# maciejkula/sbr-rs

Hardware: AMD Instinct MI355X
Metric: train interactions/sec (higher is better)
Workload: dtype f32

## Files before the change

sbr_rs_amd/csrc/sbr_device.h:

```cpp
#ifndef SBR_DEVICE_H
#define SBR_DEVICE_H

#include <hip/hip_runtime.h>

#include "../../include/sbr_hip.h"
#include "sbr_kernels.h"
#include "sbr_numerics.h"

namespace sbr {

typedef float f32x16 __attribute__((ext_vector_type(16)));

__device__ __forceinline__ float4 ld4(const float* p) { return *reinterpret_cast<const float4*>(p); }
__device__ __forceinline__ void st4(float* p, float4 v) { *reinterpret_cast<float4*>(p) = v; }
typedef float v4f_nt __attribute__((ext_vector_type(4)));
__device__ __forceinline__ float4 ld4s(const float* p) {
    const v4f_nt v = __builtin_nontemporal_load(reinterpret_cast<const v4f_nt*>(p));
    return make_float4(v.x, v.y, v.z, v.w);
}
__device__ __forceinline__ void st4s(float* p, float4 v) {
    v4f_nt t; t.x = v.x; t.y = v.y; t.z = v.z; t.w = v.w;
    __builtin_nontemporal_store(t, reinterpret_cast<v4f_nt*>(p));
}

typedef unsigned v2u __attribute__((ext_vector_type(2)));
template <int CTRL>
__device__ __forceinline__ float dpp_read(float p) {
    return __uint_as_float(__builtin_amdgcn_update_dpp(0u, __float_as_uint(p), CTRL, 0xF, 0xF, true));
}
template <int L>
__device__ __forceinline__ float group_allreduce(float p) {
    if constexpr (L >= 64) {
        const v2u r = __builtin_amdgcn_permlane32_swap(__float_as_uint(p), __float_as_uint(p), false, false);
        p = __uint_as_float(r.x) + __uint_as_float(r.y);
    }
    if constexpr (L >= 32) {
        const v2u r = __builtin_amdgcn_permlane16_swap(__float_as_uint(p), __float_as_uint(p), false, false);
        p = __uint_as_float(r.x) + __uint_as_float(r.y);
    }
    if constexpr (L >= 16) p = p + dpp_read<0x128>(p);
    if constexpr (L >= 8) {
        unsigned t = __builtin_amdgcn_update_dpp(0u, __float_as_uint(p), 0x104, 0xF, 0x5, false);
        t = __builtin_amdgcn_update_dpp(t, __float_as_uint(p), 0x114, 0xF, 0xA, false);
        p = p + __uint_as_float(t);
    }
    if constexpr (L >= 4) p = p + dpp_read<0x4E>(p);
    if constexpr (L >= 2) p = p + dpp_read<0xB1>(p);
    return p;
}
__device__ __forceinline__ void opt_update(const ModelView& m, float* w, float* acc, float* mom, float g) {
    if (m.optimizer == SBR_OPT_ADAM) sbr_adam(w, mom, acc, g, m.lr, m.l2, m.c1, m.c2);
    else sbr_adagrad(w, acc, g, m.lr, m.l2);
}


template <int D>
struct LaneGroup {
    static constexpr int L = D / 4, GPW = 64 / L;
    int lg, grp;
    uint64_t wave_first, stride;
    __device__ __forceinline__ LaneGroup(uint64_t wave = (blockIdx.x * (uint64_t)blockDim.x + threadIdx.x) >> 6,
                                         uint64_t nwaves = ((uint64_t)gridDim.x * blockDim.x) >> 6)
        : lg((int)(threadIdx.x & 63) % L), grp((int)(threadIdx.x & 63) / L), wave_first(wave * GPW), stride(nwaves * GPW) {}
    __device__ __forceinline__ uint64_t first() const { return wave_first + grp; }
};

struct EntrySource {
    uint32_t r, kind;
    __device__ __forceinline__ const float* rows(const float* dX, const float* H) const { return kind == 0 ? dX : H; }
    __device__ __forceinline__ float scale(float c) const { return kind == 0 ? 1.0f : (kind == 1 ? -c : c); }
    __device__ __forceinline__ float scale_at(const float* coef) const { return kind == 0 ? 1.0f : scale(coef[r]); }
    __device__ __forceinline__ bool carries_bias() const { return kind != 0; }
};
__device__ __forceinline__ EntrySource entry_source(uint32_t key_lo) { return EntrySource{key_lo / 3, key_lo % 3}; }

struct SeenBools {
    bool empty, hb;
    __device__ __forceinline__ SeenBools(bool any_, bool has_b_) : empty(!any_), hb(has_b_) {}
    __device__ __forceinline__ bool any() const { return !empty; }
    __device__ __forceinline__ bool has_b() const { return hb; }
};
struct SeenWord {
    uint32_t w;
    __device__ __forceinline__ SeenWord(bool any_, bool has_b_) : w((any_ ? 1u : 0u) | (has_b_ ? 2u : 0u)) {}
    __device__ __forceinline__ bool any() const { return (w & 1u) != 0; }
    __device__ __forceinline__ bool has_b() const { return (w & 2u) != 0; }
};
template <class Seen>
struct RowSumT {
    float4 g;
    float gb;
    Seen seen;
    __device__ __forceinline__ RowSumT() : g(make_float4(0.f, 0.f, 0.f, 0.f)), gb(0.0f), seen(false, false) {}
    __device__ __forceinline__ RowSumT(float4 g_, float gb_, bool any_, bool has_b_) : g(g_), gb(gb_), seen(any_, has_b_) {}
    __device__ __forceinline__ RowSumT(float4 g_, float gb_, uint32_t fl) : RowSumT(g_, gb_, (fl & 1u) != 0, (fl & 2u) != 0) {}
    __device__ __forceinline__ bool any() const { return seen.any(); }
    __device__ __forceinline__ bool has_b() const { return seen.has_b(); }
    __device__ __forceinline__ uint32_t flags() const { return (any() ? 1u : 0u) | (has_b() ? 2u : 0u); }
    __device__ __forceinline__ void add_entry(float4 v, float scale, bool carries_bias) { *this = with_entry(*this, v, scale, carries_bias); }
    template <class S2>
    __device__ __forceinline__ void add_partial(const RowSumT<S2>& o) { *this = with_partial(*this, o.g, o.gb, o.any(), o.has_b()); }

private:
    static __device__ __forceinline__ RowSumT with_entry(const RowSumT& s, float4 v, float scale, bool carries_bias) {
        float4 g = s.g;
        float gb = s.gb;
        bool empty = !s.any(), has_b = s.has_b();
        if (empty) {
            g = make_float4(scale * v.x, scale * v.y, scale * v.z, scale * v.w);
            empty = false;
        } else {
            g.x = g.x + scale * v.x; g.y = g.y + scale * v.y;
            g.z = g.z + scale * v.z; g.w = g.w + scale * v.w;
        }
        if (carries_bias) {
            gb = has_b ? gb + scale : scale;
            has_b = true;
        }
        return RowSumT(g, gb, !empty, has_b);
    }
    static __device__ __forceinline__ RowSumT with_partial(const RowSumT& s, float4 v, float vb, bool o_any, bool o_has_b) {
        float4 g = s.g;
        float gb = s.gb;
        bool empty = !s.any(), has_b = s.has_b();
        if (o_any) {
            if (empty) g = v;
            else { g.x = g.x + v.x; g.y = g.y + v.y; g.z = g.z + v.z; g.w = g.w + v.w; }
            empty = false;
        }
        if (o_has_b) {
            gb = has_b ? gb + vb : vb;
            has_b = true;
        }
        return RowSumT(g, gb, !empty, has_b);
    }
};
typedef RowSumT<SeenBools> RowSum;
typedef RowSumT<SeenWord> RowSumW;

struct PlainAccess {
    static __device__ __forceinline__ float4 ld(const float* p) { return ld4(p); }
    static __device__ __forceinline__ void st(float* p, float4 v) { st4(p, v); }
};

template <int D, bool ADAGRAD_ONLY = false>
struct RowUpdate {
    float4 w, a, mo;
    float bv, ba, bmo;
    __device__ __forceinline__ RowUpdate() : w(make_float4(0.f, 0.f, 0.f, 0.f)), a(w), mo(w), bv(0.0f), ba(0.0f), bmo(0.0f) {}
    static __device__ __forceinline__ bool adam(const ModelView& m) { return !ADAGRAD_ONLY && m.optimizer == SBR_OPT_ADAM; }
    static __device__ __forceinline__ void element(const ModelView& m, float* wv, float* acc, float* mom, float g) {
        if constexpr (ADAGRAD_ONLY) sbr_adagrad(wv, acc, g, m.lr, m.l2);
        else opt_update(m, wv, acc, mom, g);
    }
    template <class Access = PlainAccess>
    __device__ __forceinline__ void load(const ModelView& m, uint64_t row, int lg) {
        w = Access::ld(m.E + row * D + 4 * lg);
        a = Access::ld(m.Eacc + row * D + 4 * lg);
        if (adam(m)) mo = ld4(m.Em + row * D + 4 * lg);
    }
    __device__ __forceinline__ void load_bias(const ModelView& m, uint64_t row) {
        bv = m.b[row]; ba = m.bacc[row];
        if (adam(m)) bmo = m.bm[row];
    }
    template <class Sum>
    __device__ __forceinline__ void apply(const ModelView& m, const Sum& s) {
        element(m, &w.x, &a.x, &mo.x, s.g.x);
        element(m, &w.y, &a.y, &mo.y, s.g.y);
        element(m, &w.z, &a.z, &mo.z, s.g.z);
        element(m, &w.w, &a.w, &mo.w, s.g.w);
    }
    template <class Sum>
    __device__ __forceinline__ void apply_bias(const ModelView& m, const Sum& s) { element(m, &bv, &ba, &bmo, s.gb); }
    template <class Access = PlainAccess>
    __device__ __forceinline__ void store(const ModelView& m, uint64_t row, int lg) const {
        Access::st(m.E + row * D + 4 * lg, w);
        Access::st(m.Eacc + row * D + 4 * lg, a);
        if (adam(m)) st4(m.Em + row * D + 4 * lg, mo);
    }
    __device__ __forceinline__ void store_bias(const ModelView& m, uint64_t row) const {
        m.b[row] = bv;
        m.bacc[row] = ba;
        if (adam(m)) m.bm[row] = bmo;
    }
    template <class Sum>
    __device__ __forceinline__ void update_bias(const ModelView& m, uint64_t row, int lg, const Sum& s) {
        if (lg != 0 || !s.has_b()) return;
        load_bias(m, row);
        apply_bias(m, s);
        store_bias(m, row);
    }
};

template <class T>
__device__ __forceinline__ T* launder(T* p) {
    typedef T __attribute__((address_space(1))) * global_ptr;
    global_ptr g = (global_ptr)p;
    asm volatile("" : "+s"(g));
    return (T*)g;
}

__device__ __forceinline__ float dot4(float4 x, float4 y) {
    float p = x.x * y.x;
    p = sbr_fma(x.y, y.y, p);
    p = sbr_fma(x.z, y.z, p);
    p = sbr_fma(x.w, y.w, p);
    return p;
}

typedef float v2f __attribute__((ext_vector_type(2)));
__device__ __forceinline__ v2f pk_fma(v2f a, v2f b, v2f c) { return __builtin_elementwise_fma(a, b, c); }
__device__ __forceinline__ v2f pk_splat(float x) { return (v2f){x, x}; }
__device__ __forceinline__ void tanh_pq_x2(v2f x, v2f* p, v2f* q) {
    const float cx = __builtin_amdgcn_fmed3f(x.x, -SBR_TANH_CLAMP, SBR_TANH_CLAMP), cy = __builtin_amdgcn_fmed3f(x.y, -SBR_TANH_CLAMP, SBR_TANH_CLAMP);
    x.x = x.x != x.x ? x.x : cx;
    x.y = x.y != x.y ? x.y : cy;
    const v2f x2 = x * x;
    v2f n = pk_splat(-2.76076847742355e-16f);
    n = pk_fma(n, x2, pk_splat(2.00018790482477e-13f));
    n = pk_fma(n, x2, pk_splat(-8.60467152213735e-11f));
    n = pk_fma(n, x2, pk_splat(5.12229709037114e-08f));
    n = pk_fma(n, x2, pk_splat(1.48572235717979e-05f));
    n = pk_fma(n, x2, pk_splat(6.37261928875436e-04f));
    n = pk_fma(n, x2, pk_splat(4.89352455891786e-03f));
    *p = n * x;
    v2f dq = pk_splat(1.19825839466702e-06f);
    dq = pk_fma(dq, x2, pk_splat(1.18534705686654e-04f));
    dq = pk_fma(dq, x2, pk_splat(2.26843463243900e-03f));
    dq = pk_fma(dq, x2, pk_splat(4.89352518554385e-03f));
    *q = dq;
}

__device__ __forceinline__ void phase_sync() {
    __builtin_amdgcn_fence(__ATOMIC_RELEASE, "workgroup");
    __syncthreads();
    __builtin_amdgcn_fence(__ATOMIC_ACQUIRE, "workgroup");
}

template <int NT>
__device__ __forceinline__ void small_tail(const MbView& mb, const BlockView& blk, const WorkView& w, const SmallTail& t, double lsum,
                                           unsigned int tsum) {
    constexpr int NMAX = 3 * SBR_SMALL_TAIL_MAX_ROWS, NW = NT / 64;
    __shared__ uint64_t ka[NMAX], kb[NMAX];
    __shared__ uint32_t s_cnt[NW];
    const int tid = threadIdx.x, lane = tid & 63, wave = tid >> 6;
    const int R = mb.R;
    const uint32_t n = 3u * (uint32_t)R;
    __builtin_amdgcn_fence(__ATOMIC_RELEASE, "agent");
    __syncthreads();
    __builtin_amdgcn_fence(__ATOMIC_ACQUIRE, "agent");
    if (wave == 0) {
        const int ns = mb.steps[0];
        const float x = t.lag_state[1 + 2 * (ns - 1)];
        float sum = 0.0f;
        for (int base = 0; base < ns; base += 64) {
            const int tt = base + lane;
            const float v = tt < ns ? w.loss[mb.off[tt]] : 0.0f;
            const int cnt = ns - base < 64 ? ns - base : 64;
            float mine = 0.0f;
            for (int l = 0; l < cnt; ++l) {
                sum = sum + __uint_as_float(__builtin_amdgcn_readlane(__float_as_uint(v), l));
                mine = lane == l ? sum : mine;
            }
            if (tt < ns) t.lag_state[1 + 2 * tt] = mine;
        }
        if (lane == 0) {
            t.header[0] = (uint32_t)R;
            t.header[1] = tsum;
            t.header[2] = t.header[3] = 0;
            *reinterpret_cast<double*>(t.header + 4) = lsum;
            *reinterpret_cast<unsigned long long*>(t.header + 6) = (unsigned long long)R;
            if (t.loss_acc) {
                t.loss_acc[0] += lsum;
                t.loss_acc[1] += lsum;
                t.ex_acc[0] += (unsigned long long)R;
                t.ex_acc[1] += tsum;
                t.ex_acc[2] += (unsigned long long)R;
            }
            t.lag_state[0] = t.lag_state[0] + x;
        }
    }
    for (uint32_t e = tid; e < n; e += NT) {
        const uint32_t r = e / 3u, kind = e - 3u * r;
        const uint32_t* a = kind == 0 ? blk.in_idx : (kind == 1 ? blk.out_idx : blk.neg);
        ka[e] = ((uint64_t)a[r] << 32) | e;
    }
    __syncthreads();
    for (uint32_t e = tid; e < n; e += NT) {
        const uint64_t k = ka[e];
        uint32_t rank = 0;
        for (uint32_t j = 0; j < n; ++j) rank += ka[j] < k ? 1u : 0u;
        kb[rank] = k;
    }
    __syncthreads();
    const uint64_t lt = (1ull << lane) - 1ull;
    uint32_t base_heads = 0;
    for (uint32_t p0 = 0; p0 < n; p0 += NT) {
        const uint32_t p = p0 + tid;
        const bool valid = p < n;
        const bool head = valid && (p == 0 || (uint32_t)(kb[p] >> 32) != (uint32_t)(kb[p - 1] >> 32));
        if (valid) t.keys_sorted[p] = kb[p];
        const uint64_t mm = __ballot(head);
        if (lane == 0) s_cnt[wave] = (uint32_t)__popcll(mm);
        __syncthreads();
        uint32_t off = base_heads, total = 0;
#pragma unroll
        for (int w2 = 0; w2 < NW; ++w2) {
            if (w2 < wave) off += s_cnt[w2];
            total += s_cnt[w2];
        }
        if (head) t.head_pos[off + (uint32_t)__popcll(mm & lt)] = p;
        base_heads += total;
        __syncthreads();
    }
    if (tid == 0) {
        *t.nheads = base_heads;
        t.head_pos[base_heads] = n;
    }
}

}

#define DISPATCH_D(d, ...)                                         \
    switch (d) {                                                   \
        case 16: { constexpr int DD = 16; __VA_ARGS__; } break;    \
        case 32: { constexpr int DD = 32; __VA_ARGS__; } break;    \
        case 64: { constexpr int DD = 64; __VA_ARGS__; } break;    \
        case 128: { constexpr int DD = 128; __VA_ARGS__; } break;  \
        case 256: { constexpr int DD = 256; __VA_ARGS__; } break;  \
        default: break;                                            \
    }
#define DISPATCH_NQ(ndev, ...)                                           \
    do {                                                                 \
        if ((ndev) <= 4) { constexpr int NQ = 4; __VA_ARGS__; }          \
        else if ((ndev) <= 8) { constexpr int NQ = 8; __VA_ARGS__; }     \
        else { constexpr int NQ = 16; __VA_ARGS__; }                     \
    } while (0)
#endif
```

sbr_rs_amd/csrc/sbr_kernels.hip:

```cpp

#include "sbr_kernels.h"

#include <atomic>
#include <cstdlib>
#include <cstring>

#include "../../include/sbr_hip.h"
#include "sbr_device.h"
#include "sbr_numerics.h"

namespace sbr {

typedef float f32x4 __attribute__((ext_vector_type(4)));
typedef unsigned v4u32 __attribute__((ext_vector_type(4)));

#define EWMA_CHUNK_SEQS 256
#ifndef SBR_FWD_RT
#define SBR_FWD_RT 4
#endif
#ifndef SBR_FWD_WPE
#define SBR_FWD_WPE 3
#endif
#define SBR_MAX_T 1024
#ifndef SBR_FWD_RT4_MIN_TILES
// ... 1748 lines not shown
    const int nslabs = (nr + SLAB - 1) / SLAB;
    float bias_acc = 0.0f;
    const bool do_bias = tk == 0 && tid < 128;
    fetch(0);
    for (int slab = 0; slab < nslabs; ++slab) {
#pragma unroll
        for (int i = 0; i < NI; ++i) {
            st4(&Xs[(srow + 8 * i) * 128 + c4], xr[i]);
            st4(&Zs[(srow + 8 * i) * 128 + c4], zr[i]);
        }
        __syncthreads();
        fetch(slab + 1 < nslabs ? slab + 1 : slab);
        const float* xa = &Xs[hh * 128 + wk * 64 + l31];
        const float* zb = &Zs[hh * 128 + wj * 64 + l31];
        float a0 = xa[0], a1 = xa[32], b0 = zb[0], b1 = zb[32];
#pragma unroll
        for (int s = 0; s < SLAB / 2; ++s) {
            const int sn = s + 1 < SLAB / 2 ? s + 1 : s;
            const float na0 = xa[sn * 256], na1 = xa[sn * 256 + 32];
            const float nb0 = zb[sn * 256], nb1 = zb[sn * 256 + 32];
            acc[0][0] = __builtin_amdgcn_mfma_f32_32x32x2f32(a0, b0, acc[0][0], 0, 0, 0);
            acc[0][1] = __builtin_amdgcn_mfma_f32_32x32x2f32(a0, b1, acc[0][1], 0, 0, 0);
            acc[1][0] = __builtin_amdgcn_mfma_f32_32x32x2f32(a1, b0, acc[1][0], 0, 0, 0);
            acc[1][1] = __builtin_amdgcn_mfma_f32_32x32x2f32(a1, b1, acc[1][1], 0, 0, 0);
            a0 = na0; a1 = na1; b0 = nb0; b1 = nb1;
        }
        if (do_bias) {
            const int rows_here = nr - slab * SLAB < SLAB ? nr - slab * SLAB : SLAB;
            for (int r = 0; r < rows_here; ++r) bias_acc = bias_acc + Zs[r * 128 + tid];
        }
        __syncthreads();
    }
    if (do_bias) w.partials[((size_t)c * (K2 + 1) + K2) * NGD + tj * 128 + tid] = bias_acc;
    float* part = w.partials + (size_t)c * (K2 + 1) * NGD;
#pragma unroll
    for (int a = 0; a < 2; ++a)
#pragma unroll
        for (int b = 0; b < 2; ++b) {
            const int j = tj * 128 + wj * 64 + b * 32 + l31;
#pragma unroll
            for (int q = 0; q < 16; ++q) {
                const int k = tk * 128 + wk * 64 + a * 32 + (q & 3) + 8 * (q >> 2) + 4 * hh;
                part[(size_t)k * NGD + j] = acc[a][b][q];
            }
        }
}

__global__ void dense_reduce_local_kernel(const float* partials, int nchunks, size_t n, float* dense) {
    const size_t i = (size_t)blockIdx.x * blockDim.x + threadIdx.x;
    if (i >= n) return;
    float acc = partials[i];
    int c = 1;
    for (; c + 8 <= nchunks; c += 8) {
        float v[8];
#pragma unroll
        for (int j = 0; j < 8; ++j) v[j] = partials[(size_t)(c + j) * n + i];
#pragma unroll
        for (int j = 0; j < 8; ++j) acc = acc + v[j];
    }
    for (; c < nchunks; ++c) acc = acc + partials[(size_t)c * n + i];
    dense[i] = acc;
}

__device__ __forceinline__ size_t wp_index(int k, int jcol, int D, int NG) {
    const int K2 = 2 * D;
    const int g = jcol / D, u = jcol % D;
    const int ut = u >> 4, j16 = u & 15;
    const int S = k >> 4, sub = (k & 15) >> 2, kq = k & 3;
    const int lane = kq * 16 + j16;
    return ((((size_t)(ut * NG + g) * (K2 / 16) + S) * 64 + lane) * 4 + sub);
}
__device__ __forceinline__ size_t wtp_index(int k, int jcol, int D, int NG) {
    const int NGD = NG * D;
    const int ct = k >> 4, c16 = k & 15;
    const int S = jcol >> 4, sub = (jcol & 15) >> 2, kq = jcol & 3;
    const int lane = kq * 16 + c16;
    return ((((size_t)ct * (NGD / 16) + S) * 64 + lane) * 4 + sub);
}

__device__ __forceinline__ void dense_apply_element(const ModelView& m, size_t i, float g);
__global__ void dense_apply_kernel(ModelView m, const uint8_t* all_blocks, uint64_t block_bytes, uint64_t dense_off,
                                   int ndev, size_t n, const float* partials, int nchunks, float* dense_out) {
    const size_t i = (size_t)blockIdx.x * blockDim.x + threadIdx.x;
    if (i >= n) return;
    float g;
    if (partials) {
        g = partials[i];
        int c = 1;
        for (; c + 8 <= nchunks; c += 8) {
            float v[8];
#pragma unroll
            for (int j = 0; j < 8; ++j) v[j] = partials[(size_t)(c + j) * n + i];
#pragma unroll
            for (int j = 0; j < 8; ++j) g = g + v[j];
        }
        for (; c < nchunks; ++c) g = g + partials[(size_t)c * n + i];
        dense_out[i] = g;
    } else {
        g = reinterpret_cast<const float*>(all_blocks + dense_off)[i];
        for (int q = 1; q < ndev; ++q) g = g + reinterpret_cast<const float*>(all_blocks + (size_t)q * block_bytes + dense_off)[i];
    }
    dense_apply_element(m, i, g);
}
__device__ __forceinline__ void dense_apply_element(const ModelView& m, size_t i, float g) {
    if (m.ng) {
        const int NGD = m.ng * m.d;
        const size_t nw = (size_t)2 * m.d * NGD;
        if (i < nw) {
            const bool adam = m.optimizer == SBR_OPT_ADAM;
            float wv = m.W[i], G = m.Wacc[i], M = adam ? m.Wm[i] : 0.0f;
            opt_update(m, &wv, &G, &M, g);
            m.W[i] = wv;
            m.Wacc[i] = G;
            if (adam) m.Wm[i] = M;
            const int k = (int)(i / NGD), jcol = (int)(i % NGD);
            m.Wp[wp_index(k, jcol, m.d, m.ng)] = wv;
            m.WTp[wtp_index(k, jcol, m.d, m.ng)] = wv;
        } else {
            const size_t j = i - nw;
            const bool adam = m.optimizer == SBR_OPT_ADAM;
            float wv = m.bW[j], G = m.bWacc[j], M = adam ? m.bWm[j] : 0.0f;
            opt_update(m, &wv, &G, &M, g);
            m.bW[j] = wv;
            m.bWacc[j] = G;
            if (adam) m.bWm[j] = M;
        }
    } else {
        const bool adam = m.optimizer == SBR_OPT_ADAM;
        float wv = m.alpha[i], G = m.alpha_acc[i], M = adam ? m.alpha_m[i] : 0.0f;
        opt_update(m, &wv, &G, &M, g);
        m.alpha[i] = wv;
        m.alpha_acc[i] = G;
        if (adam) m.alpha_m[i] = M;
    }
}

__global__ void repack_lstm_kernel(ModelView m) {
    const int NGD = m.ng * m.d;
    const size_t nw = (size_t)2 * m.d * NGD;
    const size_t i = (size_t)blockIdx.x * blockDim.x + threadIdx.x;
    if (i >= nw) return;
    const int k = (int)(i / NGD), jcol = (int)(i % NGD);
    const float wv = m.W[i];
    m.Wp[wp_index(k, jcol, m.d, m.ng)] = wv;
    m.WTp[wtp_index(k, jcol, m.d, m.ng)] = wv;
}


struct UpdAccess {
    static __device__ __forceinline__ float4 ld(const float* p) { return ld4_upd(p); }
    static __device__ __forceinline__ void st(float* p, float4 v) { st4_upd(p, v); }
};
struct NoPrefetch {};
struct EmitApply {
    ModelView m;
    template <int D>
    __device__ __forceinline__ RowUpdate<D> pre(uint32_t r, int lg) const {
        RowUpdate<D> q;
        q.template load<UpdAccess>(m, r, lg);
        return q;
    }
    template <int D>
    __device__ __forceinline__ void row(uint32_t r, uint64_t, int lg, const RowSum& s, RowUpdate<D> q) const {
        q.apply(m, s);
        q.template store<UpdAccess>(m, r, lg);
        q.update_bias(m, r, lg, s);
    }
};
struct EmitChunk {
    void* send;
    uint64_t S;
    template <int D>
    __device__ __forceinline__ NoPrefetch pre(uint32_t, int) const { return NoPrefetch{}; }
    template <int D>
    __device__ __forceinline__ void row(uint32_t r, uint64_t, int lg, const RowSum& s, NoPrefetch) const {
        const uint32_t S32 = (uint32_t)S, owner = r / S32;
        float* c = reinterpret_cast<float*>(send) + (uint64_t)owner * S * ((uint64_t)D + 2);
        const uint64_t lr = r - owner * S32;
        st4(c + lr * D + 4 * lg, s.g);
        if (lg == 0) {
            if (s.has_b()) c[S * D + lr] = s.gb;
            reinterpret_cast<uint32_t*>(c + S * D + S)[lr] = 1u | (s.has_b() ? 2u : 0u);
        }
    }
};
struct EmitList {
    float* G;
    float* gbl;
    uint32_t* fl;
    template <int D>
    __device__ __forceinline__ NoPrefetch pre(uint32_t, int) const { return NoPrefetch{}; }
    template <int D>
    __device__ __forceinline__ void row(uint32_t, uint64_t p, int lg, const RowSum& s, NoPrefetch) const {
        st4(G + p * D + 4 * lg, s.g);
        if (lg == 0) {
            gbl[p] = s.gb;
            fl[p] = 1u | (s.has_b() ? 2u : 0u);
        }
    }
};

template <int D>
__device__ __forceinline__ RowSum seg_accumulate(const BlockView& blk, const uint64_t* keys, uint64_t begin, uint64_t end, int lg) {
    RowSum s;
    for (uint64_t e = begin; e < end; e += 4) {
        float4 v[4];
        float sc[4];
        bool bias[4];
#pragma unroll
        for (int i = 0; i < 4; ++i) {
            v[i] = make_float4(0.f, 0.f, 0.f, 0.f);
            sc[i] = 0.0f;
            bias[i] = false;
            if (e + i < end) {
                const EntrySource src = entry_source((uint32_t)keys[e + i]);
                v[i] = ld4(src.rows(blk.dX, blk.H) + (size_t)src.r * D + 4 * lg);
                sc[i] = src.scale_at(blk.coef);
                bias[i] = src.carries_bias();
            }
        }
#pragma unroll
        for (int i = 0; i < 4; ++i)
            if (e + i < end) s.add_entry(v[i], sc[i], bias[i]);
    }
    return s;
}

template <int D, int NB>
__device__ __forceinline__ RowSum seg_accumulate_long(const BlockView& blk, const uint64_t* keys, uint64_t begin, uint64_t end, int lg) {
    RowSum s;
    const uint32_t* klo = reinterpret_cast<const uint32_t*>(keys);
    uint32_t src_n[NB];
#pragma unroll
    for (int i = 0; i < NB; ++i) src_n[i] = begin + i < end ? klo[2 * (begin + i)] : 0u;
#pragma unroll 1
    for (uint64_t e = begin; e < end; e += NB) {
        float4 v[NB];
        float sc[NB];
        EntrySource src[NB];
#pragma unroll
        for (int i = 0; i < NB; ++i) {
            src[i] = entry_source(src_n[i]);
            v[i] = make_float4(0.f, 0.f, 0.f, 0.f);
            sc[i] = 0.0f;
            if (e + i < end) {
                v[i] = ld4(src[i].rows(blk.dX, blk.H) + (size_t)src[i].r * D + 4 * lg);
                sc[i] = blk.coef[src[i].r];
            }
        }
#pragma unroll
        for (int i = 0; i < NB; ++i) src_n[i] = e + NB + i < end ? klo[2 * (e + NB + i)] : 0u;
#pragma unroll
        for (int i = 0; i < NB; ++i)
            if (e + i < end) s.add_entry(v[i], src[i].scale(sc[i]), src[i].carries_bias());
    }
    return s;
}

__device__ __forceinline__ uint64_t seg_end(const uint64_t* keys, uint64_t lo, uint64_t hi, uint32_t row) {
    while (lo < hi) {
        const uint64_t mid = lo + (hi - lo) / 2;
        if ((uint32_t)(keys[mid] >> 32) == row) lo = mid + 1; else hi = mid;
    }
    return lo;
}

template <int D, class Emit, bool INLINE_LONG>
__device__ __forceinline__ void seg_short_rows(const BlockView& blk, const uint64_t* keys, uint64_t n, const SegScratch& sc, const Emit& emit,
                                               uint32_t wave, uint32_t nwaves) {
    const LaneGroup<D> lanes(wave, nwaves);
    constexpr int L = LaneGroup<D>::L;
    const int lg = lanes.lg, gbase = lanes.grp * L;
    const uint32_t nheads = *sc.nheads;
    const uint32_t stride = (uint32_t)lanes.stride;
    uint32_t h = (uint32_t)lanes.first();
    auto head_at = [&](uint32_t hh) { return sc.head_pos[hh < nheads ? hh : nheads]; };
    auto window_key = [&](uint32_t p0, uint32_t p1) {
        const uint32_t c = p1 - p0 < (uint32_t)L ? p1 - p0 : (uint32_t)L;
        return keys[(uint32_t)lg < c ? (uint64_t)p0 + lg : ((uint64_t)p0 < n ? (uint64_t)p0 : 0)];
    };
    uint32_t p_cur = head_at(h), p_end = head_at(h + 1);
    uint32_t p_next = head_at(h + stride), p_next_end = head_at(h + stride + 1);
    uint64_t kmine = window_key(p_cur, p_end);
    for (uint32_t h0 = (uint32_t)lanes.wave_first; h0 < nheads; h0 += stride, h += stride) {
        const bool active = h < nheads;
        const uint32_t p_nn = head_at(h + 2 * stride), p_nn_end = head_at(h + 2 * stride + 1);
        const uint64_t p = p_cur;
        const uint32_t len = active ? p_end - p_cur : 0u;
        const uint32_t cnt = len < (uint32_t)L ? len : (uint32_t)L;
        const uint32_t lo = (uint32_t)kmine;
        const uint32_t row = (uint32_t)__shfl((int)(uint32_t)(kmine >> 32), gbase, 64);
        kmine = window_key(p_next, p_next_end);
        p_cur = p_next;
        p_end = p_next_end;
        p_next = p_nn;
        p_next_end = p_nn_end;
        if (INLINE_LONG && len > SBR_SEG_CHUNK) {
            const auto pre = emit.template pre<D>(row, lg);
            RowSum s = seg_accumulate_long<D, 8>(blk, keys, p, p + SBR_SEG_CHUNK, lg);
            for (uint64_t q = p + SBR_SEG_CHUNK; q < p + len; q += SBR_SEG_CHUNK)
                s.add_partial(seg_accumulate_long<D, 8>(blk, keys, q, q + SBR_SEG_CHUNK < p + len ? q + SBR_SEG_CHUNK : p + len, lg));
            emit.template row<D>(row, p, lg, s, pre);
            continue;
        }
        if (!INLINE_LONG && len > SBR_SEG_ROUTE) {
            if (lg == 0 && !sc.prelisted) {
                const uint32_t slot = atomicAdd(&sc.counters[0], 1u);
                if (slot < sc.cap) {
                    sc.long_start[slot] = (uint32_t)p;
                    sc.long_end[slot] = (uint32_t)p + len;
                }
            }
            continue;
        }
        if (!active) continue;
        const auto pre = emit.template pre<D>(row, lg);
        RowSum s;
        if (len <= (uint32_t)L) {
            for (int e = 0; e < (int)cnt; e += 4) {
                float4 v[4];
                float scl[4];
                bool bias[4];
#pragma unroll
                for (int i = 0; i < 4; ++i) {
                    v[i] = make_float4(0.f, 0.f, 0.f, 0.f);
                    scl[i] = 0.0f;
                    bias[i] = false;
                    if (e + i < (int)cnt) {
                        const EntrySource src = entry_source((uint32_t)__shfl((int)lo, gbase + e + i, 64));
                        v[i] = ld4(src.rows(blk.dX, blk.H) + (size_t)src.r * D + 4 * lg);
                        scl[i] = src.scale_at(blk.coef);
                        bias[i] = src.carries_bias();
                    }
                }
#pragma unroll
                for (int i = 0; i < 4; ++i)
                    if (e + i < (int)cnt) s.add_entry(v[i], scl[i], bias[i]);
            }
        } else {
            s = seg_accumulate<D>(blk, keys, p, p + len, lg);
        }
        emit.template row<D>(row, p, lg, s, pre);
    }
}
template <int D, class Emit, bool INLINE_LONG = false>
__global__ __launch_bounds__(256) void seg_short_kernel(BlockView blk, const uint64_t* keys, uint64_t n, SegScratch sc, Emit emit) {
    seg_short_rows<D, Emit, INLINE_LONG>(blk, keys, n, sc, emit, (uint32_t)((blockIdx.x * (uint64_t)blockDim.x + threadIdx.x) >> 6),
                                         (uint32_t)(((uint64_t)gridDim.x * blockDim.x) >> 6));
}

template <int D>
__global__ __launch_bounds__(256) void small_back_kernel(ModelView m, MbView mb, BlockView blk, WorkView w, const uint64_t* keys, uint64_t nkeys,
                                                         SegScratch sc, int dw_blocks) {
    if ((int)blockIdx.x >= dw_blocks) {
        seg_short_rows<D, EmitApply, true>(blk, keys, nkeys, sc, EmitApply{m}, (uint32_t)((((uint64_t)blockIdx.x - dw_blocks) * 256 + threadIdx.x) >> 6),
                                           (uint32_t)((((uint64_t)gridDim.x - dw_blocks) * 256) >> 6));
        return;
    }
    if (m.ng == 0) {
        const int k = threadIdx.x;
        if (k >= D) return;
        float pc = 0.0f;
        for (int b = 0; b < mb.B; ++b) pc = pc + w.dab[(size_t)b * D + k];
        const float a = sbr_sigmoidf(m.alpha[k]);
        const float g = pc * (a * (1.0f - a));
        blk.dense[k] = g;
        dense_apply_element(m, (size_t)k, g);
        return;
    }
    const int NGD = m.ng * D, K2 = 2 * D, R = mb.R;
    const size_t n = (size_t)(K2 + 1) * NGD;
    const size_t i = (size_t)blockIdx.x * 256 + threadIdx.x;
    extern __shared__ __attribute__((aligned(16))) float sb_lds[];
    float* zs = sb_lds;
    float* xs = zs + (size_t)R * NGD;
    const int kmin = (int)(((size_t)blockIdx.x * 256) / NGD);
    const int klast = (int)(((size_t)blockIdx.x * 256 + 255) / NGD);
    const int nk = (klast < K2 ? klast : K2 - 1) - kmin + 1;
    for (int idx = threadIdx.x; idx < R * NGD / 4; idx += 256) st4(zs + 4 * (size_t)idx, ld4(w.dZ + 4 * (size_t)idx));
    for (int idx = threadIdx.x; idx < nk * R; idx += 256) {
        const int kk = kmin + idx / R, r = idx % R;
        float v;
        if (kk < D) {
            v = w.X[(size_t)r * D + kk];
        } else {
            const int pr = mb.prev_row[r];
            v = pr >= 0 ? blk.H[(size_t)pr * D + (kk - D)] : 0.0f;
        }
        xs[idx] = v;
    }
    __syncthreads();
    if (i >= n) return;
    const int k = (int)(i / NGD), j = (int)(i % NGD);
    const float* zc = zs + j;
    float acc = 0.0f;
    if (k < K2) {
        const float* xc = xs + (size_t)(k - kmin) * R;
#pragma unroll 8
        for (int r = 0; r < R; ++r) acc = sbr_fma(xc[r], zc[(size_t)r * NGD], acc);
    } else {
#pragma unroll 8
        for (int r = 0; r < R; ++r) acc = acc + zc[(size_t)r * NGD];
    }
    blk.dense[i] = acc;
    dense_apply_element(m, i, acc);
}

__global__ __launch_bounds__(256) void seg_long_list_kernel(SegScratch sc) {
    const uint32_t nheads = *sc.nheads;
    for (uint32_t h = blockIdx.x * 256 + threadIdx.x; h < nheads; h += gridDim.x * 256) {
        const uint32_t p0 = sc.head_pos[h], p1 = sc.head_pos[h + 1];
        if (p1 - p0 > SBR_SEG_ROUTE) {
            const uint32_t slot = atomicAdd(&sc.counters[0], 1u);
            if (slot < sc.cap) {
                sc.long_start[slot] = p0;
                sc.long_end[slot] = p1;
            }
        }
    }
}

__global__ void seg_units_kernel(SegScratch sc) {
    __shared__ uint32_t s_sum[256];
    const uint32_t nlong = sc.counters[0] < sc.cap ? sc.counters[0] : sc.cap;
    const uint32_t per = (nlong + 255) / 256;
    const uint32_t lo = threadIdx.x * per, hi = lo + per < nlong ? lo + per : nlong;
    uint32_t local = 0;
    for (uint32_t i = lo; i < hi; ++i) local += (sc.long_end[i] - sc.long_start[i] + SBR_SEG_CHUNK - 1) / SBR_SEG_CHUNK;
    s_sum[threadIdx.x] = local;
    __syncthreads();
    if (threadIdx.x == 0) {
        uint32_t run = 0;
        for (int t = 0; t < 256; ++t) { const uint32_t v = s_sum[t]; s_sum[t] = run; run += v; }
        sc.counters[1] = run;
        sc.unit_base[nlong] = run;
    }
    __syncthreads();
    uint32_t run = s_sum[threadIdx.x];
    for (uint32_t i = lo; i < hi; ++i) {
        sc.unit_base[i] = run;
        run += (sc.long_end[i] - sc.long_start[i] + SBR_SEG_CHUNK - 1) / SBR_SEG_CHUNK;
    }
}

template <int D>
__global__ __launch_bounds__(256, 6) void seg_chunk_kernel(BlockView blk, const uint64_t* keys, SegScratch sc) {
    const LaneGroup<D> lanes;
    const int lg = lanes.lg;
    const uint32_t nlong = sc.counters[0] < sc.cap ? sc.counters[0] : sc.cap;
    const uint32_t units = sc.counters[1];
    for (uint64_t u = lanes.first(); u < units; u += lanes.stride) {
        uint32_t lo = 0, hi = nlong;
        while (hi - lo > 1) {
            const uint32_t mid = lo + (hi - lo) / 2;
            if (sc.unit_base[mid] <= u) lo = mid; else hi = mid;
        }
        const uint64_t begin = (uint64_t)sc.long_start[lo] + (u - sc.unit_base[lo]) * SBR_SEG_CHUNK;
        const uint64_t end = begin + SBR_SEG_CHUNK < sc.long_end[lo] ? begin + SBR_SEG_CHUNK : sc.long_end[lo];
        const RowSum s = seg_accumulate_long<D, 4>(blk, keys, begin, end, lg);
        st4(sc.P + u * D + 4 * lg, s.g);
        if (lg == 0) {
            sc.Pb[u] = s.gb;
            sc.Pf[u] = s.has_b() ? 1u : 0u;
        }
    }
}

template <int D, class Emit>
__global__ __launch_bounds__(256) void seg_finish_kernel(const uint64_t* keys, SegScratch sc, Emit emit) {
    const LaneGroup<D> lanes;
    const int lg = lanes.lg;
    const uint32_t nlong = sc.counters[0] < sc.cap ? sc.counters[0] : sc.cap;
    for (uint64_t sidx = lanes.first(); sidx < nlong; sidx += lanes.stride) {
        const uint32_t u0 = sc.unit_base[sidx], u1 = sc.unit_base[sidx + 1];
        const bool hb0 = sc.Pf[u0] != 0;
        RowSum s(ld4(sc.P + (uint64_t)u0 * D + 4 * lg), hb0 ? sc.Pb[u0] : 0.0f, true, hb0);
        for (uint32_t u = u0 + 1; u < u1; u += 4) {
            float4 v[4];
#pragma unroll
            for (int i = 0; i < 4; ++i) v[i] = ld4(sc.P + (uint64_t)(u + i < u1 ? u + i : u1 - 1) * D + 4 * lg);
#pragma unroll
            for (int i = 0; i < 4; ++i) {
                if (u + i < u1) {
                    const bool hb = sc.Pf[u + i] != 0;
                    s.add_partial(RowSum(v[i], hb ? sc.Pb[u + i] : 0.0f, true, hb));
                }
            }
        }
        const uint64_t p = sc.long_start[sidx];
        const uint32_t row = (uint32_t)(keys[p] >> 32);
        emit.template row<D>(row, p, lg, s, emit.template pre<D>(row, lg));
    }
}

__device__ __forceinline__ float* chunk_ptr(void* base, uint64_t chunk, uint64_t S, int D) {
    return reinterpret_cast<float*>(base) + chunk * S * ((uint64_t)D + 2);
}
__device__ __forceinline__ const float* chunk_ptr(const void* base, uint64_t chunk, uint64_t S, int D) {
    return reinterpret_cast<const float*>(base) + chunk * S * ((uint64_t)D + 2);
}

__global__ void clear_chunk_flags_kernel(void* buf, int nchunks, uint64_t S, int D) {
    const uint64_t i = (uint64_t)blockIdx.x * blockDim.x + threadIdx.x;
    if (i >= (uint64_t)nchunks * S) return;
    float* c = chunk_ptr(buf, i / S, S, D);
    reinterpret_cast<uint32_t*>(c + S * D + S)[i % S] = 0u;
}

// ... 476 lines not shown
            if (m.ng == 4) {
                constexpr int ROWS = 16 * BwdCfg<DD, 4>::RT;
                hipLaunchKernelGGL((lstm_bwd_cell_kernel<DD, 4>), dim3(cell_blocks), dim3(256), 0, s, m, mb, t, blk, w);
                hipLaunchKernelGGL((lstm_bwd_gemm_kernel<DD, 4>), dim3((bt + ROWS - 1) / ROWS, (2 * DD / 16) / CTW), dim3(256), 0, s, m, mb, t, blk, w);
            } else {
                constexpr int ROWS = 16 * BwdCfg<DD, 3>::RT;
                hipLaunchKernelGGL((lstm_bwd_cell_kernel<DD, 3>), dim3(cell_blocks), dim3(256), 0, s, m, mb, t, blk, w);
                hipLaunchKernelGGL((lstm_bwd_gemm_kernel<DD, 3>), dim3((bt + ROWS - 1) / ROWS, (2 * DD / 16) / CTW), dim3(256), 0, s, m, mb, t, blk, w);
            }
        });
    }
}

int launch_dense_gradient(const ModelView& m, const MbView& mb, const BlockView& blk, const WorkView& w_in, int rows_host,
                          int b_host, hipStream_t s, bool defer_reduce) {
    if (rows_host == 0) return 0;
    if (m.ng == 0) {
        const int nch = (b_host + EWMA_CHUNK_SEQS - 1) / EWMA_CHUNK_SEQS;
        if (nch == 1) {
            hipLaunchKernelGGL(ewma_dab_final_kernel, dim3(1), dim3(m.d < 64 ? 64 : m.d), 0, s, w_in.dab, b_host, m.d, m.alpha, blk.dense);
            return 0;
        }
        hipLaunchKernelGGL(ewma_dab_chunk_kernel, dim3(nch), dim3(m.d < 64 ? 64 : m.d), 0, s, w_in.dab, b_host, m.d, w_in.partials);
        hipLaunchKernelGGL(ewma_dense_final_kernel, dim3(1), dim3(m.d < 64 ? 64 : m.d), 0, s, w_in.partials, nch, m.d, m.alpha, blk.dense);
        return 0;
    }
    const int nch = (rows_host + SBR_DW_CHUNK_ROWS - 1) / SBR_DW_CHUNK_ROWS;
    const int K2 = 2 * m.d, NGD = m.ng * m.d;
    const int tiles = ((K2 + 127) / 128) * ((NGD + 127) / 128);
    WorkView w = w_in;
    if (nch == 1) w.partials = blk.dense;
    const bool block_form = launch_wave_dense_gradient(m, mb, blk, w, rows_host, s);
    if (!block_form) DISPATCH_D(m.d, {
        const unsigned grid = (unsigned)(((nch + 7) / 8) * tiles * 8);
        constexpr bool full4 = (2 * DD) % 128 == 0 && (4 * DD) % 128 == 0, full3 = (2 * DD) % 128 == 0 && (3 * DD) % 128 == 0;
        const bool buffer_path = DD >= 128 && !w.wide_addresses && (size_t)rows_host * DD * 4 < ((size_t)1 << 31);
        const size_t pad_rows = buffer_path ? 0 : (size_t)nch * SBR_DW_CHUNK_ROWS - (size_t)rows_host;
        constexpr int lds_pad = SBR_DW_LDS_PAD;
        if (m.ng == 4) {
            if constexpr (full4) {
                if (pad_rows) (void)hipMemsetAsync(w.dZ + (size_t)rows_host * NGD, 0, pad_rows * NGD * sizeof(float), s);
                hipLaunchKernelGGL((lstm_dw_full_kernel<DD, 4>), dim3(grid), dim3(256), lds_pad, s, m, mb, blk, w);
            } else {
                hipLaunchKernelGGL((lstm_dw_kernel<DD, 4>), dim3(grid), dim3(256), 0, s, m, mb, blk, w);
            }
        } else {
            if constexpr (full3) {
                if (pad_rows) (void)hipMemsetAsync(w.dZ + (size_t)rows_host * NGD, 0, pad_rows * NGD * sizeof(float), s);
                hipLaunchKernelGGL((lstm_dw_full_kernel<DD, 3>), dim3(grid), dim3(256), 0, s, m, mb, blk, w);
            } else {
                hipLaunchKernelGGL((lstm_dw_kernel<DD, 3>), dim3(grid), dim3(256), 0, s, m, mb, blk, w);
            }
        }
    });
    if (nch == 1) return 0;
    if (defer_reduce) return nch;
    launch_dense_reduce(m, w, nch, blk, s);
    return 0;
}

void launch_dense_reduce(const ModelView& m, const WorkView& w, int nchunks, const BlockView& blk, hipStream_t s) {
    const size_t n = (size_t)(2 * m.d + 1) * m.ng * m.d;
    hipLaunchKernelGGL(dense_reduce_local_kernel, dim3((unsigned)((n + 255) / 256)), dim3(256), 0, s, w.partials, nchunks, n, blk.dense);
}

void launch_dense_apply(const ModelView& m, const uint8_t* all_blocks, uint64_t block_bytes, uint64_t dense_off,
                        int ndev, hipStream_t s) {
    const size_t n = m.ng ? (size_t)(2 * m.d + 1) * m.ng * m.d : (size_t)m.d;
    hipLaunchKernelGGL(dense_apply_kernel, dim3((unsigned)((n + 255) / 256)), dim3(256), 0, s, m, all_blocks, block_bytes, dense_off, ndev, n,
                       (const float*)nullptr, 0, (float*)nullptr);
}

void launch_dense_reduce_apply(const ModelView& m, const WorkView& w, int nchunks, const BlockView& blk, hipStream_t s) {
    const size_t n = (size_t)(2 * m.d + 1) * m.ng * m.d;
    hipLaunchKernelGGL(dense_apply_kernel, dim3((unsigned)((n + 255) / 256)), dim3(256), 0, s, m, (const uint8_t*)nullptr, (uint64_t)0, (uint64_t)0, 1, n,
                       (const float*)w.partials, nchunks, blk.dense);
}

void launch_repack_lstm(const ModelView& m, hipStream_t s) {
    if (!m.ng) return;
    const size_t nw = (size_t)2 * m.d * m.ng * m.d;
    hipLaunchKernelGGL(repack_lstm_kernel, dim3((unsigned)((nw + 255) / 256)), dim3(256), 0, s, m);
}

#ifndef SBR_SEG_INLINE_MAX_KEYS
#define SBR_SEG_INLINE_MAX_KEYS 4096
#endif
template <class Emit>
static void launch_seg_reduce(int d, const BlockView& blk, uint32_t rows_host, const uint64_t* keys_sorted, const SegScratch& sc,
                              const Emit& emit, hipStream_t s) {
    if (rows_host == 0) return;
    const uint64_t total = 3ull * rows_host;
    if (total <= SBR_SEG_INLINE_MAX_KEYS) {
        DISPATCH_D(d, {
            constexpr int gpb = groups_per_block<DD>();
            hipLaunchKernelGGL((seg_short_kernel<DD, Emit, true>), dim3(grid_for_groups((long long)total / 2 + 1, gpb)), dim3(256), 0, s, blk,
                               keys_sorted, total, sc, emit);
        });
        return;
    }
    if (!sc.prelisted) (void)hipMemsetAsync(sc.counters, 0, 2 * sizeof(uint32_t), s);
    DISPATCH_D(d, {
        constexpr int gpb = groups_per_block<DD>();
        constexpr int seg_grid_cap = 1024;
        int seg_grid = grid_for_groups((long long)total / 2 + 1, gpb);
        if (seg_grid > seg_grid_cap) seg_grid = seg_grid_cap;
        hipLaunchKernelGGL((seg_short_kernel<DD, Emit>), dim3(seg_grid), dim3(256), 0, s, blk, keys_sorted, total, sc, emit);
        if (sc.prelisted) return;
        hipLaunchKernelGGL(seg_units_kernel, dim3(1), dim3(256), 0, s, sc);
        hipLaunchKernelGGL((seg_chunk_kernel<DD>), dim3(1024), dim3(256), 0, s, blk, keys_sorted, sc);
        hipLaunchKernelGGL((seg_finish_kernel<DD, Emit>), dim3(64), dim3(256), 0, s, keys_sorted, sc, emit);
    });
}

#ifndef SBR_SMALL_BACK_MAX_ROWS
#define SBR_SMALL_BACK_MAX_ROWS 256
#endif
bool small_back_shape_ok(const ModelView& m, int rows_host) {
    if ((m.d != 16 && m.d != 32) || rows_host <= 0) return false;
    if (m.ng == 0) return 3ull * (uint64_t)rows_host <= SBR_SEG_INLINE_MAX_KEYS;
    return rows_host <= SBR_SMALL_BACK_MAX_ROWS;
}
void launch_small_back(const ModelView& m, const MbView& mb, const BlockView& blk, const WorkView& w, uint32_t rows_host,
                       const uint64_t* keys_sorted, const SegScratch& sc, hipStream_t s) {
    const size_t n = m.ng ? (size_t)(2 * m.d + 1) * m.ng * m.d : (size_t)m.d;
    const int dw_blocks = (int)((n + 255) / 256);
    const uint64_t total = 3ull * rows_host;
    DISPATCH_D(m.d, {
        if constexpr (DD <= 32) {
            constexpr int gpb = groups_per_block<DD>();
            const int seg_blocks = grid_for_groups((long long)total / 2 + 1, gpb);
            const size_t lds = m.ng ? ((size_t)rows_host * m.ng * DD + (size_t)(256 / (m.ng * DD) + 2) * rows_host) * 4 : 0;
            static std::atomic<size_t> granted[64];
            int dev = 0;
            (void)hipGetDevice(&dev);
            dev = dev >= 0 && dev < 64 ? dev : 0;
            if (lds > granted[dev]) {
                (void)hipFuncSetAttribute(reinterpret_cast<const void*>(small_back_kernel<DD>), hipFuncAttributeMaxDynamicSharedMemorySize, (int)lds);
                granted[dev] = lds;
            }
            hipLaunchKernelGGL((small_back_kernel<DD>), dim3(dw_blocks + seg_blocks), dim3(256), lds, s, m, mb, blk, w, keys_sorted, total, sc, dw_blocks);
        }
    });
}

void launch_seg_prelist(const SegScratch& sc, hipStream_t s) {
    (void)hipMemsetAsync(sc.counters, 0, 2 * sizeof(uint32_t), s);
    hipLaunchKernelGGL(seg_long_list_kernel, dim3(256), dim3(256), 0, s, sc);
    hipLaunchKernelGGL(seg_units_kernel, dim3(1), dim3(256), 0, s, sc);
}
void launch_seg_hot_apply(const ModelView& m, const BlockView& blk, const uint64_t* keys_sorted, const SegScratch& sc, hipStream_t s) {
    DISPATCH_D(m.d, {
        hipLaunchKernelGGL((seg_chunk_kernel<DD>), dim3(1024), dim3(256), 0, s, blk, keys_sorted, sc);
        hipLaunchKernelGGL((seg_finish_kernel<DD, EmitApply>), dim3(64), dim3(256), 0, s, keys_sorted, sc, EmitApply{m});
    });
}

void launch_seg_apply(const ModelView& m, const BlockView& blk, uint32_t rows_host, const uint64_t* keys_sorted,
                      const SegScratch& sc, hipStream_t s) {
    launch_seg_reduce(m.d, blk, rows_host, keys_sorted, sc, EmitApply{m}, s);
}

void launch_accumulate_loss(const uint8_t* all_blocks, uint64_t block_bytes, int ndev, double* loss_acc,
                            unsigned long long* ex_acc, hipStream_t s) {
    hipLaunchKernelGGL(accumulate_loss_kernel, dim3(1), dim3(64), 0, s, all_blocks, block_bytes, ndev, loss_acc, ex_acc);
}

void launch_seg_scatter(const ModelView& m, const BlockView& blk, uint32_t rows_host, int ndev, uint64_t slice_rows,
                        void* send, const uint64_t* keys_sorted, const SegScratch& sc, hipStream_t s) {
    const uint64_t nflags = (uint64_t)ndev * slice_rows;
    hipLaunchKernelGGL(clear_chunk_flags_kernel, dim3((unsigned)((nflags + 255) / 256)), dim3(256), 0, s, send, ndev, slice_rows, m.d);
    launch_seg_reduce(m.d, blk, rows_host, keys_sorted, sc, EmitChunk{send, slice_rows}, s);
}

void launch_owner_reduce(const ModelView& m, const ChunkPtrs& recv, int ndev, uint64_t slice_rows, void* own, hipStream_t s) {
    DISPATCH_D(m.d, {
        constexpr int gpb = groups_per_block<DD>();
        const dim3 grid(grid_for_groups((long long)slice_rows, gpb));
        DISPATCH_NQ(ndev, hipLaunchKernelGGL((owner_reduce_kernel<DD, NQ>), grid, dim3(256), 0, s, recv, ndev, slice_rows, own));
    });
}

void launch_owner_update(const ModelView& m, const ChunkPtrs& recv, int ndev, uint64_t slice_rows, uint64_t row0, uint64_t nrows, hipStream_t s) {
    if (nrows == 0) return;
    DISPATCH_D(m.d, {
        constexpr int gpb = groups_per_block<DD>();
        const dim3 grid(grid_for_groups((long long)nrows, gpb));
        DISPATCH_NQ(ndev, hipLaunchKernelGGL((owner_update_kernel<DD, NQ>), grid, dim3(256), 0, s, m, recv, ndev, slice_rows, row0, nrows));
    });
}

void launch_table_apply(const ModelView& m, const ChunkPtrs& table, uint64_t slice_rows, hipStream_t s) {
    DISPATCH_D(m.d, {
        constexpr int gpb = groups_per_block<DD>();
        hipLaunchKernelGGL((table_apply_kernel<DD>), dim3(grid_for_groups((long long)m.num_items, gpb)), dim3(256), 0, s, m, table, slice_rows);
    });
}

void launch_seg_list(const ModelView& m, const BlockView& blk, uint32_t rows_host, int ndev, uint64_t slice_rows,
                     const uint64_t* keys_sorted, float* G, float* gbl, uint32_t* fl, uint32_t* bounds, const SegScratch& sc,
                     hipStream_t s) {
    (void)hipMemsetAsync(fl, 0, (size_t)(3ull * rows_host) * sizeof(uint32_t), s);
    launch_seg_reduce(m.d, blk, rows_host, keys_sorted, sc, EmitList{G, gbl, fl}, s);
    hipLaunchKernelGGL(owner_bounds_kernel, dim3(1), dim3(64), 0, s, keys_sorted, (uint32_t)(3ull * rows_host), ndev, slice_rows, bounds);
}

void launch_owner_list_apply(const ModelView& m, const PeerLists& pl_in, const PeerBounds& pb, int ndev, int owner, MergePlan* plan,
                             uint32_t capacity, uint64_t* mkeys, uint64_t* mkeys_sorted, void* sort_temp, size_t sort_temp_bytes, hipStream_t s) {
    if (capacity == 0) return;
    PeerLists pl = pl_in;
    pl.plan = plan;
    hipLaunchKernelGGL(merge_plan_kernel, dim3(1), dim3(64), 0, s, pb, ndev, owner, plan);
    launch_merge_sort(pl, ndev, capacity, mkeys, mkeys_sorted, sort_temp, sort_temp_bytes, s);
    DISPATCH_D(m.d, {
        constexpr int gpb = groups_per_block<DD>();
        int grid = grid_for_groups((long long)capacity, gpb);
        if (grid > 2048) grid = 2048;
        DISPATCH_NQ(ndev, hipLaunchKernelGGL((owner_list_apply_kernel<DD, NQ>), dim3(grid), dim3(256), 0, s, m, pl, mkeys_sorted));
    });
}

void launch_selftest_math(const float* x, float* out_cell_h, float* out_sig, float* out_tanh, uint64_t n, hipStream_t s) {
    hipLaunchKernelGGL(selftest_math_kernel, dim3((unsigned)((n + 255) / 256)), dim3(256), 0, s, x, out_cell_h, out_sig, out_tanh, n);
}
void launch_selftest_dot_tree(const float* x, const float* y, int d, uint64_t nrows, float* out, hipStream_t s) {
    DISPATCH_D(d, {
        constexpr int gpb = groups_per_block<DD>();
        hipLaunchKernelGGL((selftest_dot_tree_kernel<DD>), dim3((unsigned)((nrows + gpb - 1) / gpb)), dim3(256), 0, s, x, y, nrows, out);
    });
}
void launch_selftest_mfma_chain(const float* a, const float* b, const float* c0, int k, float* out, hipStream_t s) {
    hipLaunchKernelGGL(selftest_mfma_chain_kernel, dim3(1), dim3(64), 0, s, a, b, c0, k, out);
}
void launch_selftest_mfma32_chain(const float* a, const float* b, int k, float* out, hipStream_t s) {
    hipLaunchKernelGGL(selftest_mfma32_chain_kernel, dim3(1), dim3(64), 0, s, a, b, k, out);
}
void launch_stream_delay(unsigned long long ticks, hipStream_t s) {
    hipLaunchKernelGGL(stream_delay_kernel, dim3(1), dim3(64), 0, s, ticks, 16384u);
}
void launch_selftest_store(float* dst, float v, hipStream_t s) {
    hipLaunchKernelGGL(selftest_store_kernel, dim3(1), dim3(64), 0, s, dst, v);
}

}
```

Measured before the change: 104.9 million.

## Batch per-row bias updates into a wave-local LDS list in segment reduce

Instead of having lane 0 of each lane group load, update and store a row's bias scalars right after the row's embedding update, the short-segment reducer now pushes (row, gradient) pairs into a per-wave shared-memory list using ballot and mbcnt. It flushes the list when full so that up to 64 lanes apply bias updates in parallel. This is meant to replace scattered single-lane scalar read-modify-writes with one coalesced batch per wave. It also adds an Adagrad-only template specialization chosen at launch, plus an environment-variable cap on list size. The cost is extra LDS use, wave barriers, and extra shuffles in the loop.

```diff
diff --git a/sbr_rs_amd/csrc/sbr_device.h b/sbr_rs_amd/csrc/sbr_device.h
--- a/sbr_rs_amd/csrc/sbr_device.h
+++ b/sbr_rs_amd/csrc/sbr_device.h
@@ -171,7 +171,8 @@
         element(m, &w.w, &a.w, &mo.w, s.g.w);
     }
     template <class Sum>
-    __device__ __forceinline__ void apply_bias(const ModelView& m, const Sum& s) { element(m, &bv, &ba, &bmo, s.gb); }
+    __device__ __forceinline__ void apply_bias(const ModelView& m, const Sum& s) { apply_bias_term(m, s.gb); }
+    __device__ __forceinline__ void apply_bias_term(const ModelView& m, float gb) { element(m, &bv, &ba, &bmo, gb); }
     template <class Access = PlainAccess>
     __device__ __forceinline__ void store(const ModelView& m, uint64_t row, int lg) const {
         Access::st(m.E + row * D + 4 * lg, w);
@@ -191,6 +192,50 @@
         store_bias(m, row);
     }
 };
+
+template <int D, bool ADAGRAD_ONLY>
+struct BiasList {
+    static constexpr uint32_t SLOTS = 64, GPW = 64 / (D / 4);
+    uint32_t* rows;
+    float* gbs;
+    uint32_t n, cap;
+    static __device__ __forceinline__ uint32_t cap_from(uint32_t request) { return request < GPW ? GPW : (request > SLOTS ? SLOTS : request); }
+    __device__ __forceinline__ BiasList(uint32_t cap_request) : n(0), cap(cap_from(cap_request)) {
+        __shared__ __attribute__((aligned(16))) uint32_t s_rows[4 * SLOTS];
+        __shared__ __attribute__((aligned(16))) float s_gbs[4 * SLOTS];
+        rows = s_rows + (threadIdx.x >> 6) * SLOTS;
+        gbs = s_gbs + (threadIdx.x >> 6) * SLOTS;
+    }
+    static __device__ __forceinline__ void wave_order() {
+        __builtin_amdgcn_fence(__ATOMIC_RELEASE, "wavefront");
+        __builtin_amdgcn_wave_barrier();
+        __builtin_amdgcn_fence(__ATOMIC_ACQUIRE, "wavefront");
+    }
+    __device__ __forceinline__ void push(const ModelView& m, bool want, uint32_t row, float gb) {
+        if (n + GPW > cap) flush(m);
+        const unsigned long long mask = __ballot(want);
+        if (want) {
+            const uint32_t slot = n + __builtin_amdgcn_mbcnt_hi((uint32_t)(mask >> 32), __builtin_amdgcn_mbcnt_lo((uint32_t)mask, 0u));
+            rows[slot] = row;
+            gbs[slot] = gb;
+        }
+        n += (uint32_t)__popcll(mask);
+    }
+    __device__ __forceinline__ void flush(const ModelView& m) {
+        wave_order();
+        const uint32_t lane = threadIdx.x & 63;
+        if (lane < n) {
+            const uint32_t row = rows[lane];
+            RowUpdate<D, ADAGRAD_ONLY> q;
+            q.load_bias(m, row);
+            q.apply_bias_term(m, gbs[lane]);
+            q.store_bias(m, row);
+        }
+        wave_order();
+        n = 0;
+    }
+};
+struct NoBiasList {};
 
 template <class T>
 __device__ __forceinline__ T* launder(T* p) {
diff --git a/sbr_rs_amd/csrc/sbr_kernels.hip b/sbr_rs_amd/csrc/sbr_kernels.hip
--- a/sbr_rs_amd/csrc/sbr_kernels.hip
+++ b/sbr_rs_amd/csrc/sbr_kernels.hip
@@ -1924,20 +1924,48 @@
     static __device__ __forceinline__ void st(float* p, float4 v) { st4_upd(p, v); }
 };
 struct NoPrefetch {};
+template <bool ADAGRAD_ONLY>
 struct EmitApply {
     ModelView m;
+    uint32_t bias_list_cap;
     template <int D>
-    __device__ __forceinline__ RowUpdate<D> pre(uint32_t r, int lg) const {
-        RowUpdate<D> q;
+    __device__ __forceinline__ RowUpdate<D, ADAGRAD_ONLY> pre(uint32_t r, int lg) const {
+        RowUpdate<D, ADAGRAD_ONLY> q;
         q.template load<UpdAccess>(m, r, lg);
         return q;
     }
     template <int D>
-    __device__ __forceinline__ void row(uint32_t r, uint64_t, int lg, const RowSum& s, RowUpdate<D> q) const {
+    __device__ __forceinline__ void row_elements(uint32_t r, int lg, const RowSum& s, RowUpdate<D, ADAGRAD_ONLY> q) const {
         q.apply(m, s);
         q.template store<UpdAccess>(m, r, lg);
+    }
+    template <int D>
+    __device__ __forceinline__ void row(uint32_t r, uint64_t, int lg, const RowSum& s, RowUpdate<D, ADAGRAD_ONLY> q) const {
+        row_elements<D>(r, lg, s, q);
         q.update_bias(m, r, lg, s);
     }
+};
+template <int D, class Emit>
+struct SegBias {
+    typedef NoBiasList List;
+    static __device__ __forceinline__ List list(const Emit&) { return List(); }
+    template <class Pre>
+    static __device__ __forceinline__ void row(const Emit& emit, uint32_t r, uint64_t p, int lg, const RowSum& s, const Pre& pre) {
+        emit.template row<D>(r, p, lg, s, pre);
+    }
+    static __device__ __forceinline__ void push(const Emit&, List&, bool, uint32_t, float) {}
+    static __device__ __forceinline__ void flush(const Emit&, List&) {}
+};
+template <int D, bool ADAGRAD_ONLY>
+struct SegBias<D, EmitApply<ADAGRAD_ONLY>> {
+    typedef EmitApply<ADAGRAD_ONLY> Emit;
+    typedef BiasList<D, ADAGRAD_ONLY> List;
+    static __device__ __forceinline__ List list(const Emit& emit) { return List(emit.bias_list_cap); }
+    static __device__ __forceinline__ void row(const Emit& emit, uint32_t r, uint64_t, int lg, const RowSum& s, const RowUpdate<D, ADAGRAD_ONLY>& pre) {
+        emit.template row_elements<D>(r, lg, s, pre);
+    }
+    static __device__ __forceinline__ void push(const Emit& emit, List& l, bool want, uint32_t r, float gb) { l.push(emit.m, want, r, gb); }
+    static __device__ __forceinline__ void flush(const Emit& emit, List& l) { l.flush(emit.m); }
 };
 struct EmitChunk {
     void* send;
@@ -2046,6 +2074,8 @@
     const uint32_t nheads = *sc.nheads;
     const uint32_t stride = (uint32_t)lanes.stride;
     uint32_t h = (uint32_t)lanes.first();
+    typedef SegBias<D, Emit> Bias;
+    typename Bias::List bias_list = Bias::list(emit);
     auto head_at = [&](uint32_t hh) { return sc.head_pos[hh < nheads ? hh : nheads]; };
     auto window_key = [&](uint32_t p0, uint32_t p1) {
         const uint32_t c = p1 - p0 < (uint32_t)L ? p1 - p0 : (uint32_t)L;
@@ -2067,15 +2097,8 @@
         p_end = p_next_end;
         p_next = p_nn;
         p_next_end = p_nn_end;
-        if (INLINE_LONG && len > SBR_SEG_CHUNK) {
-            const auto pre = emit.template pre<D>(row, lg);
-            RowSum s = seg_accumulate_long<D, 8>(blk, keys, p, p + SBR_SEG_CHUNK, lg);
-            for (uint64_t q = p + SBR_SEG_CHUNK; q < p + len; q += SBR_SEG_CHUNK)
-                s.add_partial(seg_accumulate_long<D, 8>(blk, keys, q, q + SBR_SEG_CHUNK < p + len ? q + SBR_SEG_CHUNK : p + len, lg));
-            emit.template row<D>(row, p, lg, s, pre);
-            continue;
-        }
-        if (!INLINE_LONG && len > SBR_SEG_ROUTE) {
+        const bool routed = !INLINE_LONG && len > SBR_SEG_ROUTE;
+        if (routed) {
             if (lg == 0 && !sc.prelisted) {
                 const uint32_t slot = atomicAdd(&sc.counters[0], 1u);
                 if (slot < sc.cap) {
@@ -2083,37 +2106,47 @@
                     sc.long_end[slot] = (uint32_t)p + len;
                 }
             }
-            continue;
-        }
-        if (!active) continue;
-        const auto pre = emit.template pre<D>(row, lg);
-        RowSum s;
-        if (len <= (uint32_t)L) {
-            for (int e = 0; e < (int)cnt; e += 4) {
-                float4 v[4];
-                float scl[4];
-                bool bias[4];
-#pragma unroll
-                for (int i = 0; i < 4; ++i) {
-                    v[i] = make_float4(0.f, 0.f, 0.f, 0.f);
-                    scl[i] = 0.0f;
-                    bias[i] = false;
-                    if (e + i < (int)cnt) {
-                        const EntrySource src = entry_source((uint32_t)__shfl((int)lo, gbase + e + i, 64));
-                        v[i] = ld4(src.rows(blk.dX, blk.H) + (size_t)src.r * D + 4 * lg);
-                        scl[i] = src.scale_at(blk.coef);
-                        bias[i] = src.carries_bias();
+        }
+        bool has_b = false;
+        float gb = 0.0f;
+        if (active && !routed) {
+            const auto pre = emit.template pre<D>(row, lg);
+            RowSum s;
+            if (INLINE_LONG && len > SBR_SEG_CHUNK) {
+                s = seg_accumulate_long<D, 8>(blk, keys, p, p + SBR_SEG_CHUNK, lg);
+                for (uint64_t q = p + SBR_SEG_CHUNK; q < p + len; q += SBR_SEG_CHUNK)
+                    s.add_partial(seg_accumulate_long<D, 8>(blk, keys, q, q + SBR_SEG_CHUNK < p + len ? q + SBR_SEG_CHUNK : p + len, lg));
+            } else if (len <= (uint32_t)L) {
+                for (int e = 0; e < (int)cnt; e += 4) {
+                    float4 v[4];
+                    float scl[4];
+                    bool bias[4];
+#pragma unroll
+                    for (int i = 0; i < 4; ++i) {
+                        v[i] = make_float4(0.f, 0.f, 0.f, 0.f);
+                        scl[i] = 0.0f;
+                        bias[i] = false;
+                        if (e + i < (int)cnt) {
+                            const EntrySource src = entry_source((uint32_t)__shfl((int)lo, gbase + e + i, 64));
+                            v[i] = ld4(src.rows(blk.dX, blk.H) + (size_t)src.r * D + 4 * lg);
+                            scl[i] = src.scale_at(blk.coef);
+                            bias[i] = src.carries_bias();
+                        }
                     }
+#pragma unroll
+                    for (int i = 0; i < 4; ++i)
+                        if (e + i < (int)cnt) s.add_entry(v[i], scl[i], bias[i]);
                 }
-#pragma unroll
-                for (int i = 0; i < 4; ++i)
-                    if (e + i < (int)cnt) s.add_entry(v[i], scl[i], bias[i]);
-            }
-        } else {
-            s = seg_accumulate<D>(blk, keys, p, p + len, lg);
-        }
-        emit.template row<D>(row, p, lg, s, pre);
-    }
+            } else {
+                s = seg_accumulate<D>(blk, keys, p, p + len, lg);
+            }
+            Bias::row(emit, row, p, lg, s, pre);
+            has_b = lg == 0 && s.has_b();
+            gb = s.gb;
+        }
+        Bias::push(emit, bias_list, has_b, row, gb);
+    }
+    Bias::flush(emit, bias_list);
 }
 template <int D, class Emit, bool INLINE_LONG = false>
 __global__ __launch_bounds__(256) void seg_short_kernel(BlockView blk, const uint64_t* keys, uint64_t n, SegScratch sc, Emit emit) {
@@ -2125,7 +2158,7 @@
 __global__ __launch_bounds__(256) void small_back_kernel(ModelView m, MbView mb, BlockView blk, WorkView w, const uint64_t* keys, uint64_t nkeys,
                                                          SegScratch sc, int dw_blocks) {
     if ((int)blockIdx.x >= dw_blocks) {
-        seg_short_rows<D, EmitApply, true>(blk, keys, nkeys, sc, EmitApply{m}, (uint32_t)((((uint64_t)blockIdx.x - dw_blocks) * 256 + threadIdx.x) >> 6),
+        seg_short_rows<D, EmitApply<false>, true>(blk, keys, nkeys, sc, EmitApply<false>{m, BiasList<D, false>::SLOTS}, (uint32_t)((((uint64_t)blockIdx.x - dw_blocks) * 256 + threadIdx.x) >> 6),
                                            (uint32_t)((((uint64_t)gridDim.x - dw_blocks) * 256) >> 6));
         return;
     }
@@ -2908,13 +2941,20 @@
 void launch_seg_hot_apply(const ModelView& m, const BlockView& blk, const uint64_t* keys_sorted, const SegScratch& sc, hipStream_t s) {
     DISPATCH_D(m.d, {
         hipLaunchKernelGGL((seg_chunk_kernel<DD>), dim3(1024), dim3(256), 0, s, blk, keys_sorted, sc);
-        hipLaunchKernelGGL((seg_finish_kernel<DD, EmitApply>), dim3(64), dim3(256), 0, s, keys_sorted, sc, EmitApply{m});
+        hipLaunchKernelGGL((seg_finish_kernel<DD, EmitApply<false>>), dim3(64), dim3(256), 0, s, keys_sorted, sc, EmitApply<false>{m, 0u});
     });
+}
+
+static uint32_t seg_bias_list_cap() {
+    const char* e = std::getenv("SBR_SEG_BIAS_LIST");
+    const long v = e && *e ? std::strtol(e, nullptr, 10) : 0;
+    return v > 0 && v < 64 ? (uint32_t)v : 64u;
 }
 
 void launch_seg_apply(const ModelView& m, const BlockView& blk, uint32_t rows_host, const uint64_t* keys_sorted,
                       const SegScratch& sc, hipStream_t s) {
-    launch_seg_reduce(m.d, blk, rows_host, keys_sorted, sc, EmitApply{m}, s);
+    if (m.optimizer == SBR_OPT_ADAM) launch_seg_reduce(m.d, blk, rows_host, keys_sorted, sc, EmitApply<false>{m, seg_bias_list_cap()}, s);
+    else launch_seg_reduce(m.d, blk, rows_host, keys_sorted, sc, EmitApply<true>{m, seg_bias_list_cap()}, s);
 }
 
 void launch_accumulate_loss(const uint8_t* all_blocks, uint64_t block_bytes, int ndev, double* loss_acc,
```

Result: no change. 105.6 million (median of 6 runs) (+0.7%).
